# ohsnyt/bzip2-rust

Hardware: AMD Instinct MI355X
Metric: compress MB/s at -9 (900 KB blocks), 1/2/4/8 MI355X; bit-exact vs C bzip2 (higher is better)
Workload: dtype u8; 1 GPU; 1024 MiB per GPU synthetic text at -9 (1194 blocks on this rank), BASELINE configs[2]; raw_bytes_total=1073741824, blocks_rank0=1194, compressed_bytes=323302688

## Files before the change

bzip2-rust_amd/csrc/bzx_api.hip:

```cpp
#include <string.h>
#include <chrono>
#include <new>
#include "bzx_host.h"
#include "bzx_wg.h"

extern "C" const char *bzx_version(void) { return "bzx 0.1 (gfx950)"; }

extern "C" const char *bzx_strerror(int code)
{
    switch (code) {
    case BZX_OK: return "ok";
    case BZX_E_NODEVICE: return "no HIP device";
    case BZX_E_PARAM: return "bad parameter";
    case BZX_E_NOMEM: return "out of memory";
    case BZX_E_OUTBUF: return "output buffer too small";
    case BZX_E_HIP: return "HIP runtime error";
    case BZX_E_STATE: return "bad call sequence";
    case BZX_E_DATA: return "damaged or invalid bzip2 data";
    default: return "unknown error";
    }
}

extern "C" const char *bzx_last_error(const bzx_ctx *ctx) { return ctx ? ctx->err.c_str() : ""; }

// ... 989 lines not shown
}

extern "C" int bzx_split_rle1_chunk(bzx_ctx *ctx, const uint8_t *raw, size_t len, int level, int final, uint8_t *blocks_out,
                                    uint32_t nblk_cap, uint32_t *ns, uint32_t *crcs, uint32_t *nblk_out)
{
    auto api_lock_ = ctx_lock(ctx);
    BZX_REFUSE_WHILE_STREAMING(ctx);
    if (!ctx || !blocks_out || !ns || !crcs || !nblk_out || !level_ok(level) || (len && !raw)) return BZX_E_PARAM;
    HIP_TRY(ctx, hipSetDevice(ctx->device));
    *nblk_out = 0;
    std::vector<uint8_t> &carry = ctx->split_carry;
    const size_t total = carry.size() + len;
    uint32_t use = 0;
    uint64_t last_start = 0;
    int rc = split_to_host(ctx, carry.data(), carry.size(), raw, len, level, final, blocks_out, nblk_cap, ns, crcs, &use,
                           &last_start);
    if (rc) return rc;
    std::vector<uint8_t> next;
    if (!final) {
        const size_t ls = (size_t)last_start, cs = carry.size();
        try {
            next.reserve(total - ls);
            if (ls < cs) next.insert(next.end(), carry.begin() + ls, carry.end());
            const size_t from = ls > cs ? ls - cs : 0;
            if (len > from) next.insert(next.end(), raw + from, raw + len);
        } catch (const std::bad_alloc &) {
            return BZX_E_NOMEM;
        }
    }
    carry.swap(next);
    *nblk_out = use;
    return BZX_OK;
}

extern "C" void *bzx_host_alloc(size_t bytes)
{
    void *p = nullptr;
    return hipHostMalloc(&p, bytes ? bytes : 1, BZX_HOST_PORTABLE) == hipSuccess ? p : nullptr;
}
extern "C" void bzx_host_free(void *p)
{
    if (p) (void)hipHostFree(p);
}


#ifdef BZX_DIAG
extern "C" int bzx_dbg_set_stop(bzx_ctx *ctx, uint32_t k)
{
    if (!ctx) return BZX_E_PARAM;
    ctx->B.dbg_stop = k;
    return BZX_OK;
}

extern "C" int bzx_dbg_phase_timers(bzx_ctx *ctx, int enable, unsigned long long out[128])
{
    if (!ctx) return BZX_E_PARAM;
    if (enable && !ctx->d_dbg) {
        if (hipMalloc((void **)&ctx->d_dbg, 128 * sizeof(unsigned long long)) != hipSuccess) return BZX_E_NOMEM;
    }
    if (out && ctx->d_dbg) {
        HIP_TRY(ctx, hipStreamSynchronize(ctx->stream));
        HIP_TRY(ctx, hipMemcpy(out, ctx->d_dbg, 128 * sizeof(unsigned long long), hipMemcpyDeviceToHost));
    }
    if (ctx->d_dbg) HIP_TRY(ctx, hipMemset(ctx->d_dbg, 0, 128 * sizeof(unsigned long long)));
    ctx->B.dbg = enable ? ctx->d_dbg : nullptr;
    return BZX_OK;
}

extern "C" int bzx_dbg_block_times(bzx_ctx *ctx, uint32_t nblk, uint32_t *us_out, uint32_t *n_out, uint32_t *inuse_out)
{
    if (!ctx || !us_out || nblk > ctx->cap_blocks) return BZX_E_PARAM;
    HIP_TRY(ctx, hipStreamSynchronize(ctx->stream));
    HIP_TRY(ctx, hipMemcpy(ctx->h_blk, ctx->B.blk, nblk * sizeof(BzxBlock), hipMemcpyDeviceToHost));
    for (uint32_t b = 0; b < nblk; b++) {
        us_out[b] = ctx->h_blk[b].pad_[1];
        if (n_out) n_out[b] = ctx->h_blk[b].n;
        if (inuse_out) inuse_out[b] = ctx->h_blk[b].n_in_use;
    }
    return BZX_OK;
}
#endif
```

bzip2-rust_amd/csrc/bzx_bsort.hip:

```cpp
#include <hip/hip_runtime.h>
#include "bzx_host.h"
#include "bzx_wg.h"
#include "bzx_pack.h"

#define BS_NT 1024
#define BS_NW (BS_NT / 64)
#ifndef BS_C
#define BS_C 2048
#endif
#define BS_FW (BS_C / 64)
#define BS_ISO (BS_C / 3)
#ifndef BS_ISO_SHIFT
#define BS_ISO_SHIFT 5
#endif
#ifndef BS_BIN1
#define BS_BIN1 15
#endif
#define BS_BIN2 12
#define BS_NBIN1 (1u << BS_BIN1)
#define BS_TAB_WORDS (BS_NBIN1 + (BS_NBIN1 >> 5))
#define BS_MAX_BK 1024
#ifndef BS_MAX_BIG
#define BS_MAX_BIG 512
#endif
#define SP_U 4
#ifndef BS_MAX_DEPTH
#define BS_MAX_DEPTH 511
#endif
#ifndef BS_MAX_SPLITS
#define BS_MAX_SPLITS 1024
#endif
#ifndef BS_ROUNDS
#define BS_ROUNDS 4
#endif
#ifndef BS_KEYBITS
#define BS_KEYBITS 32
#endif
#define BS_TINY 64
#define BS_MED 512
#define REC_IDX(r) ((uint32_t)((r) >> 12) & 0xFFFFFu)
#define REC_PREV(r) ((uint32_t)((r) >> 4) & 0xFFu)
#define W_POS_MASK 0x3FFFull

static_assert(BS_C <= 16384, "bucket capacity");

#ifdef BZX_DIAG
__shared__ unsigned long long s_diag[128];
#define DIAG_T0()                                                             \
    unsigned long long t_last_ = 0;                                           \
    if (B.dbg && threadIdx.x == 0) {                                          \
        for (int i_ = 0; i_ < 128; i_++) s_diag[i_] = 0;                      \
        t_last_ = wall_clock64();                                             \
    }                                                                         \
    (void)t_last_;
#define DIAG_STAMP(slot)                                                      \
    do {                                                                      \
        if (B.dbg && threadIdx.x == 0) {                                      \
            const unsigned long long now_ = wall_clock64();                   \
            s_diag[slot] += now_ - t_last_;                                   \
            t_last_ = now_;                                                   \
        }                                                                     \
    } while (0)
#define DIAG_COUNT(slot, v)                                                   \
    do {                                                                      \
        if (B.dbg && threadIdx.x == 0) s_diag[slot] += (unsigned long long)(v); \
    } while (0)
#define DIAG_FLUSH()                                                          \
    do {                                                                      \
        if (B.dbg && threadIdx.x == 0)                                        \
            for (int i_ = 0; i_ < 128; i_++)                                  \
                if (s_diag[i_]) atomicAdd(&B.dbg[i_], s_diag[i_]);            \
    } while (0)
#else
#define DIAG_T0() do {} while (0)
#define DIAG_STAMP(slot) do {} while (0)
#define DIAG_COUNT(slot, v) do {} while (0)
#define DIAG_FLUSH() do {} while (0)
#endif

__shared__ uint32_t b_tab[BS_TAB_WORDS + BS_MAX_BK];
__shared__ uint32_t b_start[BS_MAX_BK + 1];
__shared__ uint32_t b_first[BS_MAX_BK + 1];
__shared__ uint32_t b_cur[BS_MAX_BK];
__shared__ uint8_t b_b0[BS_MAX_BK];
__shared__ uint32_t b_inuse[256];
__shared__ uint8_t b_seq[256];
__shared__ uint32_t b_scratch[2 * BS_NW];
__shared__ uint32_t b_lbase[8];
__shared__ uint32_t b_bcast[12];
__shared__ uint32_t b_big[BS_MAX_BIG][3];

#define TAB(b) b_tab[(b) + ((b) >> 5)]

template <int ISO, int PER>
__device__ __forceinline__ void bucket_flags(const uint32_t (&c)[PER], uint32_t bin0, uint32_t excl, uint32_t prevc, uint32_t &fl, uint32_t &nf)
{
    constexpr uint32_t CP = BS_C - ISO;
    uint32_t s = excl, ps = excl - prevc, pc = prevc;
#pragma unroll
    for (int k = 0; k < PER; k++) {
        const bool f = (bin0 + k == 0) || c[k] > (uint32_t)ISO || pc > (uint32_t)ISO || (s / CP != ps / CP);
        fl |= (uint32_t)f << k;
        nf += f;
        ps = s;
        s += c[k];
        pc = c[k];
    }
}

template <int BINS, bool TAB16 = false>
__device__ __forceinline__ uint32_t form_buckets(uint32_t total)
{
    constexpr int PER = BINS / BS_NT;
    const uint32_t tid = threadIdx.x, bin0 = tid * PER;
    uint32_t c[PER], sum = 0, e8 = 0, e6 = 0, e4 = 0;
#pragma unroll
    for (int k = 0; k < PER; k++) {
        c[k] = TAB(bin0 + k);
        sum += c[k];
        const uint32_t m = c[k] <= BS_ISO ? c[k] : 0u;
        e8 += m > BS_C / 8 ? m : 0u;
        e6 += m > BS_C / 6 ? m : 0u;
        e4 += m > BS_C / 4 ? m : 0u;
    }
    const uint32_t prevc = tid ? TAB(bin0 - 1) : 0u;
    if (__any(e8 != 0)) {
// ... 428 lines not shown
{
    const uint32_t tid = threadIdx.x, lvl = B.deep_lvl;
    const uint32_t listed = B.counters[BZX_CTR_DEEP_CNT + lvl];
    const uint32_t n_items = listed < B.deep_cap ? listed : B.deep_cap;
    if (n_items == 0) return;
    DIAG_T0();
    const BzxDeepItem *list = reinterpret_cast<const BzxDeepItem *>(B.deep_list) + (size_t)(lvl & 1u) * B.deep_cap;
    for (;;) {
        if (tid == 0) b_bcast[0] = atomicAdd(&B.counters[BZX_CTR_DEEP_FETCH + lvl], 1u);
        __syncthreads();
        const uint32_t i = b_bcast[0];
        __syncthreads();
        if (i >= n_items) break;
        const BzxDeepItem d = list[i];
        if (d.cnt == 0) continue;
        const uint32_t b = d.blk;
        if (__atomic_load_n(&B.blk[b].status, __ATOMIC_RELAXED) & BZX_ST_REDO) continue;
        const uint32_t n = B.blk[b].n, bits = d.dbits >> 16;
        const size_t sb = BZX_SLAB(B, b);
        const uint8_t *__restrict__ P = B.pk + sb * BZX_PK_STRIDE;
        uint64_t *__restrict__ rec_a = B.rec_a + sb * BZX_MAX_N;
        uint64_t *__restrict__ rec_b = B.rec_b + sb * BZX_MAX_N;
        if (tid == 0) {
            b_bcast[3] = 1;
            b_bcast[4] = 0;
            b_big[0][0] = d.st;
            b_big[0][1] = d.cnt;
            b_big[0][2] = d.dbits & 0xFFFFu;
        }
        __syncthreads();
        const bool ok = deep_process(B, b, (b - B.blk_first) / B.blk_step, n, bits, P, rec_a, rec_b, 0, 1,
                                     lvl + 1 < BZX_DEEP_LEVELS ? (int)lvl + 1 : -1);
        if (!ok && tid == 0) block_redo(B, b);
        __syncthreads();
    }
    DIAG_FLUSH();
}

#ifndef SK_NT
#define SK_NT 256
#endif
#define SK_NW (SK_NT / 64)
#define BS_E (BS_C / SK_NT)
#define SK_DB 8
#define SK_ND (1u << SK_DB)
static_assert(BS_C % SK_NT == 0 && BS_E >= 1 && BS_E <= 8, "bucket capacity");

__shared__ uint64_t s_x[BS_C];
__shared__ __attribute__((aligned(16))) uint64_t s_w[BS_C + 4];
__shared__ __attribute__((aligned(16))) uint32_t s_cnt[SK_NW][SK_ND];
__shared__ uint32_t s_dbase[SK_ND];
__shared__ uint32_t s_part[4];
__shared__ uint64_t s_f[BS_FW + 1];
__shared__ uint32_t s_med[BS_C / BS_TINY + 1];
__shared__ uint32_t s_large[BS_C / BS_MED + 1];
__shared__ uint32_t s_rc[2][4];
__shared__ uint32_t s_bc[8];
__shared__ uint32_t s_m[2];
__shared__ uint32_t s_red[SK_NW][4];

__device__ __forceinline__ uint32_t uni(uint32_t v) { return bzx_uni(v); }
__device__ __forceinline__ uint32_t tid_here() { return bzx_tid_here(); }
__device__ __forceinline__ BzxBucket uni(BzxBucket b)
{
    BzxBucket r;
    r.blk = uni(b.blk);
    r.start = uni(b.start);
    r.cnt = uni(b.cnt);
    if (r.cnt >> 31) r.cnt = 0;
    r.dbits = uni(b.dbits);
    return r;
}

__device__ __forceinline__ void wave_rank(uint32_t *wc, uint32_t d, bool valid, uint32_t lane, uint32_t &old, uint32_t &rank)
{
    uint64_t m = __ballot(valid);
    uint32_t plo = (uint32_t)m, phi = (uint32_t)(m >> 32);
#pragma unroll
    for (int b = 0; b < SK_DB; b++) {
        const uint32_t mask = 0u - ((d >> b) & 1u);
        m = __ballot((d >> b) & 1u);
        plo &= ~((uint32_t)m ^ mask);
        phi &= ~((uint32_t)(m >> 32) ^ mask);
    }
    const uint64_t peers = ((uint64_t)phi << 32) | plo;
    rank = (uint32_t)__popcll(peers & ((1ull << lane) - 1ull));
    old = wc[d];
    lds_order();
    if (valid && rank == 0) atomicAdd(&wc[d], (uint32_t)__popcll(peers));
    lds_order();
}

__device__ __attribute__((noinline)) void wg_radix_sort(uint32_t base, uint32_t cnt, int lo, int hi)
{
    uint64_t *A = s_w + base;
    const uint32_t tid = threadIdx.x, lane = bzx_lane(), wave = bzx_wave();
    const uint32_t rows = (cnt + SK_NT - 1) / SK_NT, chunk = rows * 64;
    if (tid == 0) {
        s_bc[5] = 0;
        s_bc[6] = 0;
    }
    __syncthreads();
    {
        const uint64_t a0 = A[0];
        uint64_t d = 0;
#pragma unroll
// ... 20 lines not shown
        uint32_t old[BS_E], rk[BS_E];
#pragma unroll
        for (uint32_t j = 0; j < BS_E; j++) {
            const uint32_t e = wave * chunk + j * 64 + lane;
            v[j] = j < rows && e < cnt ? A[e] : 0ull;
        }
#pragma unroll
        for (uint32_t j = 0; j < BS_E; j++) {
            const uint32_t e = wave * chunk + j * 64 + lane;
            wave_rank(wc, (uint32_t)(v[j] >> shift) & (SK_ND - 1), j < rows && e < cnt, lane, old[j], rk[j]);
        }
        __syncthreads();
        {
            constexpr uint32_t SK_DK = SK_ND > SK_NT ? SK_ND / SK_NT : 1u;
            if (tid * SK_DK < SK_ND) {
                uint32_t tot[SK_DK], sum = 0;
#pragma unroll
                for (uint32_t i = 0; i < SK_DK; i++) {
                    uint32_t run = 0;
#pragma unroll
                    for (int w = 0; w < SK_NW; w++) {
                        const uint32_t t = s_cnt[w][tid * SK_DK + i];
                        s_cnt[w][tid * SK_DK + i] = run;
                        run += t;
                    }
                    tot[i] = run;
                    sum += run;
                }
                const uint32_t incl = bzx_wave_incl_sum(sum);
                uint32_t run = incl - sum;
#pragma unroll
                for (uint32_t i = 0; i < SK_DK; i++) {
                    s_dbase[tid * SK_DK + i] = run;
                    run += tot[i];
                }
                if (lane == 63) s_part[wave] = incl;
            }
        }
        __syncthreads();
        const uint32_t p1 = s_part[0], p2 = p1 + s_part[1], p3 = p2 + s_part[2];
#pragma unroll
        for (uint32_t j = 0; j < BS_E; j++) {
            const uint32_t e = wave * chunk + j * 64 + lane;
            if (j < rows && e < cnt) {
                const uint32_t d = (uint32_t)(v[j] >> shift) & (SK_ND - 1);
                const uint32_t q = SK_ND > SK_NT ? 0u : d >> 6;
                A[s_dbase[d] + (q == 0 ? 0u : q == 1 ? p1 : q == 2 ? p2 : p3) + wc[d] + old[j] + rk[j]] = v[j];
            }
        }
        __syncthreads();
    }
}

__device__ __attribute__((noinline)) void wg_radix_sort_opt(uint32_t cnt, int lo, int hi)
{
    uint64_t *A = s_x;
    const uint32_t lane = bzx_lane(), wave = bzx_wave();
    const uint32_t rows = (cnt + SK_NT - 1) / SK_NT, chunk = rows * 64;
    __syncthreads();
    uint64_t diff;
    {
        uint32_t o0 = 0, o1 = 0, a0 = ~0u, a1 = ~0u;
#pragma unroll
        for (int w = 0; w < SK_NW; w++) {
            o0 |= s_red[w][0];
            o1 |= s_red[w][1];
            a0 &= s_red[w][2];
            a1 &= s_red[w][3];
        }
        diff = ((uint64_t)(o1 & ~a1) << 32) | (o0 & ~a0);
    }
    uint32_t *wc = s_cnt[wave];
    uint32_t *wb = reinterpret_cast<uint32_t *>(s_w) + wave * SK_ND;
    for (int shift = lo; shift < hi; shift += SK_DB) {
        if (((diff >> shift) & (uint64_t)(SK_ND - 1)) == 0) continue;
#pragma unroll
        for (uint32_t i = 0; i < SK_ND / 64; i++) wc[i * 64 + lane] = 0;
        lds_order();
        uint64_t v[BS_E];
        uint32_t old[BS_E];
#pragma unroll
        for (uint32_t j = 0; j < BS_E; j++) {
            const uint32_t e = wave * chunk + j * 64 + lane;
            v[j] = j < rows && e < cnt ? A[e] : 0ull;
        }
#pragma unroll
        for (uint32_t j = 0; j < BS_E; j++) {
            const uint32_t e = wave * chunk + j * 64 + lane;
            old[j] = bzx_lds_ticket(&wc[(uint32_t)(v[j] >> shift) & (SK_ND - 1)], j < rows && e < cnt);
        }
        __syncthreads();
        {
            static_assert(SK_ND == 4 * 64, "four digits per lane");
            uint32_t mine[4], tot[4], sum = 0;
#pragma unroll
            for (uint32_t i = 0; i < 4; i++) mine[i] = tot[i] = 0;
#pragma unroll
            for (uint32_t w = 0; w < SK_NW; w++) {
                const uint4 c = *reinterpret_cast<const uint4 *>(&s_cnt[w][4 * lane]);
                const uint32_t cc[4] = {c.x, c.y, c.z, c.w};
#pragma unroll
                for (uint32_t i = 0; i < 4; i++) {
                    if (w < wave) mine[i] += cc[i];
                    tot[i] += cc[i];
                }
            }
#pragma unroll
            for (uint32_t i = 0; i < 4; i++) sum += tot[i];
            uint32_t run = bzx_wave_incl_sum(sum) - sum;
            uint4 o;
            o.x = run + mine[0];
            run += tot[0];
            o.y = run + mine[1];
            run += tot[1];
            o.z = run + mine[2];
            run += tot[2];
            o.w = run + mine[3];
            *reinterpret_cast<uint4 *>(&wb[4 * lane]) = o;
        }
        lds_order();
#pragma unroll
        for (uint32_t j = 0; j < BS_E; j++) {
            const uint32_t e = wave * chunk + j * 64 + lane;
            if (j < rows && e < cnt) A[wb[(uint32_t)(v[j] >> shift) & (SK_ND - 1)] + old[j]] = v[j];
        }
        __syncthreads();
    }
}

template <bool TICKETS>
__device__ __attribute__((noinline)) void wave_radix_sort(uint32_t base, uint32_t s, int lo, int hi)
{
    constexpr uint32_t ROWS = BS_MED / 64;
    uint64_t *A = s_w + base;
    uint32_t *wc = s_cnt[bzx_wave()];
    const uint32_t lane = bzx_lane();
    const uint32_t rows = (s + 63u) / 64u;
    uint64_t v[ROWS];
    uint64_t diff = 0;
    {
        const uint64_t a0 = A[0];
#pragma unroll
        for (uint32_t j = 0; j < ROWS; j++) {
            const uint32_t e = j * 64 + lane;
            v[j] = e < s ? A[e] : 0ull;
            if (e < s) diff |= v[j] ^ a0;
        }
#pragma unroll
        for (int sh = 32; sh > 0; sh >>= 1) diff |= __shfl_xor(diff, sh);
    }
    for (int shift = lo; shift < hi; shift += SK_DB) {
        if (((diff >> shift) & (uint64_t)(SK_ND - 1)) == 0) continue;
#pragma unroll
        for (uint32_t i = 0; i < SK_ND / 64; i++) wc[i * 64 + lane] = 0;
        lds_order();
        uint32_t old[ROWS], rk[ROWS];
#pragma unroll
        for (uint32_t j = 0; j < ROWS; j++) {
            old[j] = rk[j] = 0;
            if (j < rows) {
                if (TICKETS) old[j] = bzx_lds_ticket(&wc[(uint32_t)(v[j] >> shift) & (SK_ND - 1)], j * 64 + lane < s);
                else wave_rank(wc, (uint32_t)(v[j] >> shift) & (SK_ND - 1), j * 64 + lane < s, lane, old[j], rk[j]);
            }
        }
        {
            uint32_t c[SK_ND / 64], sum = 0;
#pragma unroll
            for (uint32_t i = 0; i < SK_ND / 64; i++) {
                c[i] = wc[(SK_ND / 64) * lane + i];
                sum += c[i];
            }
            uint32_t run = bzx_wave_incl_sum(sum) - sum;
            lds_order();
#pragma unroll
            for (uint32_t i = 0; i < SK_ND / 64; i++) {
                wc[(SK_ND / 64) * lane + i] = run;
                run += c[i];
            }
        }
        lds_order();
#pragma unroll
        for (uint32_t j = 0; j < ROWS; j++)
            if (j * 64 + lane < s) A[wc[(uint32_t)(v[j] >> shift) & (SK_ND - 1)] + old[j] + rk[j]] = v[j];
        lds_order();
#pragma unroll
        for (uint32_t j = 0; j < ROWS; j++) {
            const uint32_t e = j * 64 + lane;
            v[j] = e < s ? A[e] : 0ull;
        }
        lds_order();
    }
}

__device__ __forceinline__ uint32_t fbit(uint32_t p) { return (uint32_t)(s_f[p >> 6] >> (p & 63u)) & 1u; }
__device__ __forceinline__ void fset(uint32_t p) { atomicOr((unsigned long long *)&s_f[p >> 6], 1ull << (p & 63u)); }

__device__ __forceinline__ bool tiny_bounds(uint32_t p, uint32_t &gs, uint32_t &ge)
{
    const uint32_t wi = p >> 6, bi = p & 63u;
    uint64_t w = s_f[wi] & (~0ull >> (63u - bi));
    if (w) {
        gs = wi * 64 + 63u - (uint32_t)__builtin_clzll(w);
    } else {
        if (wi == 0) return false;
        w = s_f[wi - 1];
        if (!w) return false;
        gs = (wi - 1) * 64 + 63u - (uint32_t)__builtin_clzll(w);
    }
    w = bi == 63u ? 0ull : s_f[wi] & (~0ull << (bi + 1u));
    if (w) {
        ge = wi * 64 + (uint32_t)__builtin_ctzll(w);
    } else {
        w = s_f[wi + 1];
        if (!w) return false;
        ge = (wi + 1) * 64 + (uint32_t)__builtin_ctzll(w);
    }
    return ge - gs <= BS_TINY;
}

__device__ __forceinline__ void mark_changes(uint32_t base, uint32_t s, int lo, uint32_t t, uint32_t step)
{
    for (uint32_t e = 1 + t; e < s; e += step)
        if ((s_w[base + e] >> lo) != (s_w[base + e - 1] >> lo)) fset(base + e);
}

__device__ __forceinline__ bool any_big(uint32_t base, uint32_t s, uint32_t t, uint32_t step)
{
    bool big = false;
    for (uint32_t e = t; e < s; e += step) {
        uint32_t gs, ge;
        big |= !tiny_bounds(base + e, gs, ge);
    }
    return big;
}

__device__ __forceinline__ void wave_sort_mark(uint32_t base, uint32_t s, int lo, uint32_t lane)
{
    wave_radix_sort<true>(base, s, lo, 64);
    lds_order();
    uint32_t diff = 0;
    bool bad = false;
    for (uint32_t e = 1 + lane, k = 0; e < s; e += 64, k++) {
        const uint64_t a = s_w[base + e] >> lo, b = s_w[base + e - 1] >> lo;
        bad |= a < b;
        diff |= (uint32_t)(a != b) << k;
    }
// ... 122 lines not shown
                for (uint32_t k = 0; k < 4; k++) {
                    const bool in = i + k < sz;
                    r += in && wq[k] < my[j];
                    rk += in && wq[k] < myc;
                }
            }
            if (sz) dst_[j] = (a_ + r) | (r != rk ? 0u : 0x80000000u);
        }
    }
    __syncthreads();
}

__device__ __forceinline__ void place_ranked(const uint32_t (&dst_)[BS_E], const uint64_t (&my)[BS_E])
{
#pragma unroll
    for (uint32_t j = 0; j < BS_E; j++) {
        if (dst_[j] != 0xFFFFFFFFu) {
            const uint32_t q = dst_[j] & 0x7FFFFFFFu;
            s_w[q] = my[j];
            if ((dst_[j] >> 31) && !fbit(q)) fset(q);
        }
    }
    __syncthreads();
}

#define LIST(which, i) (reinterpret_cast<uint16_t *>(s_x)[4u * (i) + 2u + (which)])

template <bool ALL>
__device__ __attribute__((noinline)) void list_tied(uint32_t n, uint32_t from, uint32_t to)
{
    const uint32_t tid = tid_here(), lane = tid & 63u;
    const uint32_t nrow = (n + SK_NT - 1) / SK_NT;
#pragma unroll
    for (uint32_t j = 0; j < BS_E; j++) {
        if (j < nrow) {
            const uint32_t i = j * SK_NT + tid;
            uint32_t p = 0;
            bool t = false;
            if (i < n) {
                p = ALL ? i : (uint32_t)LIST(from, i);
                t = !(fbit(p) && fbit(p + 1));
            }
            const uint64_t mk = __ballot(t);
            if (mk) {
                uint32_t base = 0;
                if (lane == 0) base = atomicAdd(&s_m[to], (uint32_t)__popcll(mk));
                base = bzx_bcast0(base);
                if (t) LIST(to, base + (uint32_t)__popcll(mk & ((1ull << lane) - 1ull))) = (uint16_t)p;
            }
        }
    }
}

__device__ __forceinline__ bool initial_sort(uint32_t cnt)
{
    const uint32_t tid = tid_here(), lane = tid & 63u, wave = tid >> 6;
    uint64_t fm[BS_E];
    wg_radix_sort_opt(cnt, 64 - BS_KEYBITS, 64);
    int bad = 0;
#pragma unroll
    for (uint32_t j = 0; j < BS_E; j++) {
        const uint32_t p = j * SK_NT + tid;
        s_w[p] = p;
        const uint64_t kp = s_x[p] >> (64 - BS_KEYBITS), kq = p ? s_x[p - 1] >> (64 - BS_KEYBITS) : 0ull;
        const bool f = p >= cnt || p == 0 || kp != kq;
        bad |= p < cnt && p > 0 && kp < kq;
        fm[j] = __ballot(f);
        if (lane == 0) s_f[j * SK_NW + wave] = fm[j];
    }
    if (tid == 0) s_f[BS_FW] = ~0ull;
    if (__syncthreads_or(bad)) return false;
#pragma unroll
    for (uint32_t j = 0; j < BS_E; j++) {
        const uint64_t mk = tied_mask(fm[j], s_f[j * SK_NW + wave + 1]);
        if (mk) {
            uint32_t base = 0;
            if (lane == 0) base = atomicAdd(&s_m[0], (uint32_t)__popcll(mk));
            base = bzx_bcast0(base);
            if ((mk >> lane) & 1ull) LIST(0, base + (uint32_t)__popcll(mk & ((1ull << lane) - 1ull))) = (uint16_t)(j * SK_NT + tid);
        }
    }
    return true;
}

__device__ __attribute__((noinline)) uint32_t wave_rounds(const uint8_t *__restrict__ P, uint32_t bits, uint32_t nbits, uint32_t m,
                                                          uint32_t lpar, uint32_t round, uint32_t dcur)
{
    const uint32_t lane = bzx_lane();
    for (;; round++) {
        if (m == 0) return dcur;
        if (!(round < BS_ROUNDS && dcur < nbits)) return dcur | 0x80000000u;
        const bool has = lane < m;
        uint32_t p = 0, gs = 0, ge = 0;
        uint64_t my = 0;
        if (has) {
            p = LIST(lpar, lane);
            const uint32_t pos = (uint32_t)(s_w[p] & W_POS_MASK);
            uint32_t x = REC_IDX(s_x[pos]) * bits + dcur;
            if (x >= nbits) x -= nbits;
            my = (pk_window_bit(P, x) & ~W_POS_MASK) | pos;
            tiny_bounds(p, gs, ge);
        }
        lds_order();
        if (has) s_w[p] = my;
        lds_order();
        uint32_t r = 0, rk = 0;
        const uint64_t myc = my & ~W_POS_MASK;
        const uint32_t sz = ge - gs;
        for (uint32_t i = 0; __ballot(i < sz); i++) {
            if (i < sz) {
                const uint64_t o = s_w[gs + i];
                r += o < my;
                rk += o < myc;
            }
        }
        lds_order();
        if (has) {
            const uint32_t q = gs + r;
            s_w[q] = my;
            if (r == rk && !fbit(q)) fset(q);
        }
        lds_order();
        const bool t = has && !(fbit(p) && fbit(p + 1));
        const uint64_t mk = __ballot(t);
        if (t) LIST(lpar ^ 1u, (uint32_t)__popcll(mk & ((1ull << lane) - 1ull))) = (uint16_t)p;
        lds_order();
        m = (uint32_t)__popcll(mk);
        lpar ^= 1u;
        dcur += 50;
    }
}

#ifndef SK_WAVES_PER_SIMD
#define SK_WAVES_PER_SIMD 4
#endif
#ifdef BZX_HIP_EMU
#define BS_LOAD_REC(p) (*(p))
#else
#define BS_LOAD_REC(p) __builtin_nontemporal_load(p)
#endif
__device__ __forceinline__ void bsort_body(const BzxBatch &B)
{
    const uint32_t tid0 = threadIdx.x;
    if (B.bsort_mode == 1 && B.counters[BZX_CTR_RESUME] == 0) return;
    DIAG_T0();
    const uint32_t G = gridDim.x >> 3;
    const uint32_t cap8 = B.bk_cap >> 3, lx = blockIdx.x & 7u;
    const uint32_t n_lx = B.counters[BZX_CTR_BK_LIST0 + lx] < cap8 ? B.counters[BZX_CTR_BK_LIST0 + lx] : cap8;
    const uint32_t n_items = lx * cap8 + n_lx;
    uint32_t idx = lx * cap8 + (blockIdx.x >> 3);
    BzxBucket it = {0, 0, 0, 0}, nit = {0, 0, 0, 0};
    if (idx < n_items) it = uni(B.bk_list[idx]);
    if (idx + G < n_items) nit = uni(B.bk_list[idx + G]);
    uint64_t nxt[BS_E];
    uint32_t n_cur = 0, st_cur = 0;
    if (it.cnt) {
        const uint64_t *__restrict__ src = ((it.start >> 31) ? B.rec_b : B.rec_a) + BZX_SLAB(B, it.blk) * BZX_MAX_N +
                                           (it.start & 0x7fffffffu);
#pragma unroll
        for (uint32_t j = 0; j < BS_E; j++) nxt[j] = j * SK_NT + tid0 < it.cnt ? BS_LOAD_REC(src + j * SK_NT + tid0) : ~0ull;
        n_cur = uni(B.blk[it.blk].n);
        st_cur = uni(__atomic_load_n(&B.blk[it.blk].status, __ATOMIC_RELAXED));
    }
    for (; idx < n_items; idx += G) {
        BzxBucket nit2 = {0, 0, 0, 0};
        if (idx + 2 * G < n_items) nit2 = B.bk_list[idx + 2 * G];
        uint32_t tid = tid_here(), lane = tid & 63u, wave = tid >> 6;
        const uint32_t b = it.blk, cnt = it.cnt;
        const uint32_t start = it.start & 0x7fffffffu, bits = it.dbits >> 16, depth0 = it.dbits & 0xFFFFu;
        const uint8_t *__restrict__ P = B.pk + BZX_SLAB(B, b) * BZX_PK_STRIDE;
        const uint32_t nbits = n_cur * bits;
        const bool skip = cnt == 0 || (cnt >> 31) || (st_cur & BZX_ST_REDO) || (B.bsort_mode == 1 && !(st_cur & BZX_ST_RESUME));
        DIAG_STAMP(64);
        if (!skip) {
            uint32_t o0 = 0, o1 = 0, a0 = ~0u, a1 = ~0u;
#pragma unroll
            for (uint32_t j = 0; j < BS_E; j++) {
                s_x[j * SK_NT + tid] = nxt[j];
                if (j * SK_NT + tid < cnt) {
                    o0 |= (uint32_t)nxt[j];
                    o1 |= (uint32_t)(nxt[j] >> 32);
                    a0 &= (uint32_t)nxt[j];
                    a1 &= (uint32_t)(nxt[j] >> 32);
                }
            }
            o0 = bzx_wave_incl_or(o0);
            o1 = bzx_wave_incl_or(o1);
            a0 = bzx_wave_incl_and(a0);
            a1 = bzx_wave_incl_and(a1);
            if (lane == 63) {
                s_red[wave][0] = o0;
                s_red[wave][1] = o1;
                s_red[wave][2] = a0;
                s_red[wave][3] = a1;
            }
        }
        uint32_t n_nx = 0, st_nx = 0;
#define PREFETCH_NEXT()                                                                                                   \
        if (nit.cnt) {                                                                                                    \
            const uint64_t *__restrict__ src = ((nit.start >> 31) ? B.rec_b : B.rec_a) + BZX_SLAB(B, nit.blk) * BZX_MAX_N + \
                                               (nit.start & 0x7fffffffu);                                                 \
            const uint32_t tp_ = tid_here();                                                                              \
            _Pragma("unroll") for (uint32_t j = 0; j < BS_E; j++) nxt[j] = j * SK_NT + tp_ < nit.cnt ? BS_LOAD_REC(src + j * SK_NT + tp_) : ~0ull; \
            n_nx = B.blk[nit.blk].n;                                             \
            st_nx = __atomic_load_n(&B.blk[nit.blk].status, __ATOMIC_RELAXED);                                            \
        }
        if (skip) {
            PREFETCH_NEXT();
            it = nit;
            nit = uni(nit2);
            n_cur = uni(n_nx);
            st_cur = uni(st_nx);
            continue;
        }
        if (tid < 4) s_rc[0][tid] = 0;
        if (tid < 2) s_m[tid] = 0;
        DIAG_STAMP(65);
        if (!initial_sort(cnt)) {
            if (tid == 0) {
                atomicAdd(&B.counters[BZX_CTR_STAT0 + 15], 1u);
                block_redo(B, b);
            }
            PREFETCH_NEXT();
            __syncthreads();
            it = nit;
            nit = uni(nit2);
            n_cur = uni(n_nx);
            st_cur = uni(st_nx);
            continue;
        }
        DIAG_STAMP(67);

        uint32_t dcur = depth0 + BS_KEYBITS;
        bool fail = false;
        uint32_t lpar = 0;
        __syncthreads();
        DIAG_STAMP(73);
        for (uint32_t round = 0;; round++) {
            tid = tid_here();
            lane = tid & 63u;
            wave = tid >> 6;
            const uint32_t par = round & 1u;
            const uint32_t m = uni(s_m[lpar]);
            if (m == 0) break;
            if (m <= 64) {
                DIAG_COUNT(89, 1);
                if (wave == 0) {
                    dcur = wave_rounds(P, bits, nbits, m, lpar, round, dcur);
                    if (lane == 0) s_bc[3] = dcur;
                }
                __syncthreads();
                dcur = uni(s_bc[3]);
                fail = dcur >> 31;
                dcur &= 0x7FFFFFFFu;
                DIAG_STAMP(70);
                break;
            }
            if (!(round < BS_ROUNDS && dcur < nbits)) {
                DIAG_COUNT(round >= BS_ROUNDS ? 84 : 85, 1);
                fail = true;
                break;
            }
            DIAG_COUNT(80, 1);
            DIAG_COUNT(88, m);
            const uint32_t nrow = (m + SK_NT - 1) / SK_NT;
            uint32_t amask = 0, hmask = 0;
            uint32_t pq[BS_E], xa[BS_E];
#pragma unroll
            for (uint32_t j = 0; j < BS_E; j++) {
                pq[j] = 0;
                xa[j] = 0;
// ... 11 lines not shown
            for (uint32_t j = 0; j < BS_E; j++) {
                if ((amask >> j) & 1u) {
                    uint32_t x = REC_IDX(s_x[pq[j] >> 16]) * bits + dcur;
                    if (x >= nbits) x -= nbits;
                    xa[j] = x;
                }
            }
            uint64_t g[BS_E];
#pragma unroll
            for (uint32_t j = 0; j < BS_E; j++) g[j] = ((amask >> j) & 1u) ? pk_window_bit(P, xa[j]) : 0ull;
            const auto rank_of = [&](uint32_t j) { return pq[j] & 0xFFFFu; };
            list_big_groups(hmask, par, rank_of);
#pragma unroll
            for (uint32_t j = 0; j < BS_E; j++)
                if ((amask >> j) & 1u) s_w[pq[j] & 0xFFFFu] = (g[j] & ~W_POS_MASK) | (uint64_t)(pq[j] >> 16);
            if (tid == 0) {
                s_rc[par ^ 1u][0] = s_rc[par ^ 1u][1] = s_rc[par ^ 1u][2] = s_rc[par ^ 1u][3] = 0;
                s_m[lpar ^ 1u] = 0;
            }
            __syncthreads();
            DIAG_STAMP(68);
            const uint32_t nmed = s_rc[par][1], nlarge = s_rc[par][2];
            if (nmed | nlarge) {
                DIAG_COUNT(86, nmed);
                DIAG_COUNT(87, nlarge);
                sort_listed_groups(par, nmed, nlarge, tid, lane);
                DIAG_STAMP(69);
            }
            tid = tid_here();
            lane = tid & 63u;
            wave = tid >> 6;
            uint32_t dst_[BS_E];
            uint64_t my[BS_E];
            rank_tiny_groups(amask, nrow, rank_of, dst_, my);
            DIAG_STAMP(70);
            place_ranked(dst_, my);
            DIAG_STAMP(71);
            list_tied<false>(m, lpar, lpar ^ 1u);
            __syncthreads();
            DIAG_STAMP(73);
            lpar ^= 1u;
            dcur += 50;
        }
        PREFETCH_NEXT();
        tid = tid_here();
        if (fail || B.bsort_mode == 1) {
            uint64_t *__restrict__ sax = B.rec_a + BZX_SLAB(B, b) * BZX_MAX_N + start;
            const uint32_t rk = uni(B.blk[b].n_selectors);
            uint32_t *__restrict__ isa0 = rank_array(B, rk, 0), *__restrict__ isa1 = rank_array(B, rk, 1);
#pragma unroll
            for (uint32_t j = 0; j < BS_E; j++) {
                const uint32_t p = j * SK_NT + tid;
                if (p < cnt) {
                    const uint32_t rot = REC_IDX(s_x[(uint32_t)(s_w[p] & W_POS_MASK)]);
                    const uint32_t f0 = fbit(p);
                    sax[p] = (uint64_t)rot | ((uint64_t)f0 << 32);
                    if (isa0) {
                        const uint32_t head = f0 ? p : group_start(p);
                        isa0[rot] = start + head;
                        if (f0 && fbit(p + 1)) isa1[rot] = start + head;
                    }
                }
            }
            if (fail) {
                uint32_t *__restrict__ cl = reinterpret_cast<uint32_t *>(B.rec_b + BZX_SLAB(B, b) * BZX_MAX_N + start);
                uint64_t mk[BS_E];
                lane = tid & 63u;
                wave = tid >> 6;
#pragma unroll
                for (uint32_t j = 0; j < BS_E; j++) mk[j] = tied_mask(s_f[j * SK_NW + wave], s_f[j * SK_NW + wave + 1]);
                slot_counts_publish(mk, BS_E);
                __syncthreads();
                uint32_t before[BS_E];
                const uint32_t total = slot_counts_sum(BS_E, before);
#pragma unroll
                for (uint32_t j = 0; j < BS_E; j++) {
                    if ((mk[j] >> lane) & 1ull) {
                        const uint32_t p = j * SK_NT + tid;
                        const uint32_t rot = REC_IDX(s_x[(uint32_t)(s_w[p] & W_POS_MASK)]);
                        cl[before[j] + (uint32_t)__popcll(mk[j] & ((1ull << lane) - 1ull))] = p | (fbit(p) << 11) | (rot << 12);
                    }
                }
                if (tid == 0) {
                    atomicMin(&B.blk[b].n_mtf, dcur / bits);
                    B.bk_list[idx].cnt = cnt | 0x80000000u;
                    const uint32_t ri = atomicAdd(&B.counters[BZX_CTR_RK_ITEMS], 1u);
                    B.rk_list[ri] = idx;
                    B.rk_list[B.bk_cap + ri] = total;
                    atomicAdd(&B.counters[BZX_CTR_RK_OPEN], 1u);
                    atomicAdd(&B.blk[b].n_groups, 1u);
                    if ((atomicOr(&B.blk[b].status, BZX_ST_RESUME) & BZX_ST_RESUME) == 0)
                        B.resume_list[atomicAdd(&B.counters[BZX_CTR_RESUME], 1u)] = b;
                }
            }
        }
        {
            constexpr uint32_t OUT_E = 8;
            uint8_t *__restrict__ L = B.bwt + BZX_SLAB(B, b) * BZX_BLK_STRIDE + start;
            const uint32_t p0 = tid * OUT_E;
            if (p0 < cnt) {
                const uint32_t rot = tid >> 2;
                uint32_t pos[OUT_E];
#pragma unroll
                for (uint32_t k = 0; k < OUT_E; k++) pos[k] = (uint32_t)(s_w[p0 + ((k + rot) & (OUT_E - 1))] & W_POS_MASK);
                uint64_t bytes = 0;
#pragma unroll
                for (uint32_t k = 0; k < OUT_E; k++) {
                    const uint32_t kk = (k + rot) & (OUT_E - 1);
                    const uint32_t r = reinterpret_cast<const uint32_t *>(s_x)[2u * pos[k]];
                    bytes |= (uint64_t)REC_PREV(r) << (8 * kk);
                    if (p0 + kk < cnt && REC_IDX(r) == 0) B.blk[b].orig_ptr = start + p0 + kk;
                }
                if (p0 + OUT_E <= cnt) {
                    __builtin_memcpy(L + p0, &bytes, 8);
                } else {
                    for (uint32_t k = 0; p0 + k < cnt; k++) L[p0 + k] = (uint8_t)(bytes >> (8 * k));
                }
            }
            DIAG_COUNT(83, 1);
        }
        __syncthreads();
        DIAG_STAMP(72);
        it = nit;
        nit = uni(nit2);
        n_cur = uni(n_nx);
        st_cur = uni(st_nx);
    }
    DIAG_FLUSH();
}

__global__ __launch_bounds__(SK_NT, SK_WAVES_PER_SIMD) void bzx_bsort_kernel(BzxBatch B) { bsort_body(B); }
__global__ __launch_bounds__(SK_NT, SK_WAVES_PER_SIMD) void bzx_bfill_kernel(BzxBatch B) { bsort_body(B); }

#define RK_CHUNK 16
struct RkMeta {
    uint32_t bi, T, blk, start, cnt, n, rk, h0;
};
__shared__ RkMeta s_meta[RK_CHUNK];

__device__ __forceinline__ uint32_t rk_fetch_chunk(const BzxBatch &B, uint32_t n_items, uint32_t &open)
{
    __shared__ uint32_t s_fetch[2];
    __syncthreads();
    if (threadIdx.x < 64) {
        uint32_t base = 0;
        if (threadIdx.x == 0) base = atomicAdd(&B.counters[B.rk_fetch], (uint32_t)RK_CHUNK);
        base = __shfl(base, 0);
        const uint32_t i = base + threadIdx.x;
        bool op = false;
        if (threadIdx.x < RK_CHUNK && i < n_items) {
            RkMeta m;
            m.bi = B.rk_list[i];
            m.T = B.rk_list[B.bk_cap + i];
            const BzxBucket it = B.bk_list[m.bi];
            op = !(it.dbits >> 31);
            m.blk = it.blk;
            m.start = it.start & 0x7fffffffu;
            m.cnt = it.cnt & 0x7fffffffu;
            m.n = B.blk[it.blk].n;
            m.rk = B.blk[it.blk].n_selectors;
            m.h0 = B.blk[it.blk].n_mtf;
            s_meta[threadIdx.x] = m;
        }
        const uint64_t m = __ballot(op);
        if (threadIdx.x == 0) {
            s_fetch[0] = base;
            s_fetch[1] = (uint32_t)m;
        }
    }
    __syncthreads();
    open = s_fetch[1];
    return s_fetch[0];
}

__shared__ uint32_t s_stall[2 * BS_FW];

__device__ __forceinline__ void rank_round_wave(const BzxBatch &B, uint32_t i)
{
    const uint32_t lane = bzx_lane(), wave = bzx_wave();
    const RkMeta &mt = s_meta[i & (RK_CHUNK - 1)];
// ... 543 lines not shown
```

bzip2-rust_amd/csrc/bzx_device.h:

```cpp
#pragma once
#include <stdint.h>
#include <stddef.h>

#define BZX_MAX_N 900000u
#define BZX_BLK_STRIDE 900096u
#define BZX_MAX_ALPHA 258
#define BZX_G_SIZE 50
#define BZX_N_ITERS 4
#define BZX_MAX_SEL 18002
#define BZX_SEL_STRIDE 18048

#define BZX_IN_RAW (1ull << 63)
#define BZX_ST_PERIODIC 1u
#define BZX_ST_REDO 2u
#define BZX_ST_RESUME 4u
#define BZX_ST_DC_RANDOMISED 0x400u
#define DC_ERR_HEADER 0x100u
#define DC_ERR_DATA 0x200u
#define DC_SKIP 0x800u
#define DC_MAGIC_BLOCK 0x314159265359ull
#define DC_MAGIC_EOS 0x177245385090ull
#ifndef RK_ROUNDS
#define RK_ROUNDS 11
#endif
#define RK_COARSE 0x80000000u
#define BZX_PK_STRIDE 900352u
#ifndef BZX_BK_PER_BLOCK
#define BZX_BK_PER_BLOCK 2048u
#endif

#define BZX_CTR_PERIODIC 5
#define BZX_CTR_BK_LIST0 40
#ifndef BZX_DEEP_LEVELS
#define BZX_DEEP_LEVELS 2
#endif
#define BZX_DEEP_PER_BLOCK 128u
#define BZX_CTR_DEEP_CNT 48
#define BZX_CTR_DEEP_FETCH 56
#define BZX_CTR_GIANT_CNT (BZX_CTR_DEEP_CNT + BZX_DEEP_LEVELS)
#define BZX_CTR_GIANT_FETCH (BZX_CTR_DEEP_FETCH + BZX_DEEP_LEVELS)
#define BZX_CTR_BK_FETCH 9
#define BZX_CTR_REDO 10
#define BZX_CTR_SPLIT_FETCH 11
#define BZX_CTR_REDO_FETCH 12
#define BZX_CTR_RESUME 13
#define BZX_CTR_RESUME_FETCH 14
#define BZX_CTR_RK_ITEMS 32
#define BZX_CTR_RK_OPEN 33
#define BZX_CTR_RK_FETCH 64
#define BZX_N_COUNTERS 192
#define BZX_CTR_RESUME_LEFT 34
#define BZX_CTR_STAT0 16

struct BzxBucket {
    uint32_t blk;
    uint32_t start;
    uint32_t cnt;
    uint32_t dbits;
};

struct BzxBlock {
    uint64_t in_off;
    uint32_t n;
    uint32_t crc;
    uint32_t orig_ptr;
    uint32_t status;
    uint32_t n_mtf;
    uint32_t n_in_use;
    uint32_t n_groups;
    uint32_t n_selectors;
    uint64_t bits;
    uint64_t out_bit;
    uint32_t sec_bits[4];
    uint32_t pad_[2];
    uint64_t pack_word;
};

struct BzxSortWs {
    uint64_t *u0;
    uint64_t *u1;
    uint32_t *s0;
    uint32_t *s1;
    uint32_t *isa;
    uint32_t *sa;
};

struct BzxBatch {
    BzxBlock *blk;
    uint32_t nblk;
    uint32_t blk_first;
    uint32_t blk_step;
    uint32_t ctr_bwt;
    uint32_t packed;
    uint32_t *counters;
    uint32_t *plist;
    const uint8_t *in;
    const uint8_t *raw;
    uint8_t *bwt;
    uint8_t *rank;
    uint32_t *hpos;
    uint32_t hpos_stride;
    uint16_t *mtfv;
    uint32_t *freq;
// ... 93 lines not shown
```

Baseline: 29770 MB/s.

## Feed bucket-sort records from registers and skip identity position writes

The radix sort now takes the prefetched records as register arguments, so the initial store of all records to shared memory and the reload in the first pass go away. The global prefetch layout changes to wave-chunked rows so each thread already holds the elements the sort expects. A per-word 'tied' bitmap (s_t) is added so s_w position entries are written only for tied positions, and readers fall back to the identity index otherwise, which cuts LDS writes. A debug per-workgroup timer export is also added. The cost is more shared memory and a branch on every position lookup.

```diff
diff --git a/bzip2-rust_amd/csrc/bzx_api.hip b/bzip2-rust_amd/csrc/bzx_api.hip
--- a/bzip2-rust_amd/csrc/bzx_api.hip
+++ b/bzip2-rust_amd/csrc/bzx_api.hip
@@ -1065,11 +1065,20 @@
     return BZX_OK;
 }
 
+extern "C" int bzx_dbg_wg_times(bzx_ctx *ctx, unsigned long long out[BZX_DBG_WG])
+{
+    if (!ctx || !out || !ctx->d_dbg) return BZX_E_PARAM;
+    HIP_TRY(ctx, hipStreamSynchronize(ctx->stream));
+    HIP_TRY(ctx, hipMemcpy(out, ctx->d_dbg + 128, BZX_DBG_WG * sizeof(unsigned long long), hipMemcpyDeviceToHost));
+    return BZX_OK;
+}
+
 extern "C" int bzx_dbg_phase_timers(bzx_ctx *ctx, int enable, unsigned long long out[128])
 {
     if (!ctx) return BZX_E_PARAM;
     if (enable && !ctx->d_dbg) {
-        if (hipMalloc((void **)&ctx->d_dbg, 128 * sizeof(unsigned long long)) != hipSuccess) return BZX_E_NOMEM;
+        if (hipMalloc((void **)&ctx->d_dbg, (128 + BZX_DBG_WG) * sizeof(unsigned long long)) != hipSuccess) return BZX_E_NOMEM;
+        if (hipMemset(ctx->d_dbg, 0, (128 + BZX_DBG_WG) * sizeof(unsigned long long)) != hipSuccess) return BZX_E_NOMEM;
     }
     if (out && ctx->d_dbg) {
         HIP_TRY(ctx, hipStreamSynchronize(ctx->stream));
diff --git a/bzip2-rust_amd/csrc/bzx_bsort.hip b/bzip2-rust_amd/csrc/bzx_bsort.hip
--- a/bzip2-rust_amd/csrc/bzx_bsort.hip
+++ b/bzip2-rust_amd/csrc/bzx_bsort.hip
@@ -71,7 +71,16 @@
             for (int i_ = 0; i_ < 128; i_++)                                  \
                 if (s_diag[i_]) atomicAdd(&B.dbg[i_], s_diag[i_]);            \
     } while (0)
+#define DIAG_WG_TIME()                                                        \
+    do {                                                                      \
+        if (B.dbg && threadIdx.x == 0 && B.bsort_mode == 0 && blockIdx.x < BZX_DBG_WG) { \
+            unsigned long long sum_ = 0;                                      \
+            for (int i_ = 64; i_ < 74; i_++) sum_ += s_diag[i_];              \
+            B.dbg[128 + blockIdx.x] = sum_;                                   \
+        }                                                                     \
+    } while (0)
 #else
+#define DIAG_WG_TIME() do {} while (0)
 #define DIAG_T0() do {} while (0)
 #define DIAG_STAMP(slot) do {} while (0)
 #define DIAG_COUNT(slot, v) do {} while (0)
@@ -606,6 +615,7 @@
 __shared__ uint32_t s_dbase[SK_ND];
 __shared__ uint32_t s_part[4];
 __shared__ uint64_t s_f[BS_FW + 1];
+__shared__ uint64_t s_t[BS_FW];
 __shared__ uint32_t s_med[BS_C / BS_TINY + 1];
 __shared__ uint32_t s_large[BS_C / BS_MED + 1];
 __shared__ uint32_t s_rc[2][4];
@@ -732,11 +742,24 @@
     }
 }
 
-__device__ __attribute__((noinline)) void wg_radix_sort_opt(uint32_t cnt, int lo, int hi)
-{
+#ifdef BZX_HIP_EMU
+extern "C" {
+unsigned bzx_emu_bsort_nopass = 0;
+}
+#define BS_NOPASS_HOOK() do { if (threadIdx.x == 0) bzx_emu_bsort_nopass++; } while (0)
+#else
+#define BS_NOPASS_HOOK() do {} while (0)
+#endif
+
+__device__ __attribute__((noinline)) void wg_radix_sort_opt(uint32_t cnt, int lo, int hi, uint64_t x0, uint64_t x1, uint64_t x2, uint64_t x3,
+                                                            uint64_t x4, uint64_t x5, uint64_t x6, uint64_t x7)
+{
+    static_assert(BS_E == 8, "one parameter per row");
     uint64_t *A = s_x;
     const uint32_t lane = bzx_lane(), wave = bzx_wave();
     const uint32_t rows = (cnt + SK_NT - 1) / SK_NT, chunk = rows * 64;
+    uint64_t v[BS_E] = {x0, x1, x2, x3, x4, x5, x6, x7};
+    bool first = true;
     __syncthreads();
     uint64_t diff;
     {
@@ -757,13 +780,15 @@
 #pragma unroll
         for (uint32_t i = 0; i < SK_ND / 64; i++) wc[i * 64 + lane] = 0;
         lds_order();
-        uint64_t v[BS_E];
         uint32_t old[BS_E];
-#pragma unroll
-        for (uint32_t j = 0; j < BS_E; j++) {
-            const uint32_t e = wave * chunk + j * 64 + lane;
-            v[j] = j < rows && e < cnt ? A[e] : 0ull;
-        }
+        if (!first) {
+#pragma unroll
+            for (uint32_t j = 0; j < BS_E; j++) {
+                const uint32_t e = wave * chunk + j * 64 + lane;
+                v[j] = j < rows && e < cnt ? A[e] : 0ull;
+            }
+        }
+        first = false;
 #pragma unroll
         for (uint32_t j = 0; j < BS_E; j++) {
             const uint32_t e = wave * chunk + j * 64 + lane;
@@ -806,6 +831,15 @@
         }
         __syncthreads();
     }
+    if (first) {
+        BS_NOPASS_HOOK();
+#pragma unroll
+        for (uint32_t j = 0; j < BS_E; j++) {
+            const uint32_t e = wave * chunk + j * 64 + lane;
+            if (j < rows && e < cnt) A[e] = v[j];
+        }
+        __syncthreads();
+    }
 }
 
 template <bool TICKETS>
@@ -872,6 +906,10 @@
     }
 }
 
+__device__ __forceinline__ uint32_t pos_of(uint32_t p)
+{
+    return ((s_t[p >> 6] >> (p & 63u)) & 1ull) ? (uint32_t)(s_w[p] & W_POS_MASK) : p;
+}
 __device__ __forceinline__ uint32_t fbit(uint32_t p) { return (uint32_t)(s_f[p >> 6] >> (p & 63u)) & 1u; }
 __device__ __forceinline__ void fset(uint32_t p) { atomicOr((unsigned long long *)&s_f[p >> 6], 1ull << (p & 63u)); }
 
@@ -1100,16 +1138,15 @@
     }
 }
 
-__device__ __forceinline__ bool initial_sort(uint32_t cnt)
+__device__ __forceinline__ bool initial_sort(uint32_t cnt, const uint64_t (&rec)[BS_E])
 {
     const uint32_t tid = tid_here(), lane = tid & 63u, wave = tid >> 6;
     uint64_t fm[BS_E];
-    wg_radix_sort_opt(cnt, 64 - BS_KEYBITS, 64);
+    wg_radix_sort_opt(cnt, 64 - BS_KEYBITS, 64, rec[0], rec[1], rec[2], rec[3], rec[4], rec[5], rec[6], rec[7]);
     int bad = 0;
 #pragma unroll
     for (uint32_t j = 0; j < BS_E; j++) {
         const uint32_t p = j * SK_NT + tid;
-        s_w[p] = p;
         const uint64_t kp = s_x[p] >> (64 - BS_KEYBITS), kq = p ? s_x[p - 1] >> (64 - BS_KEYBITS) : 0ull;
         const bool f = p >= cnt || p == 0 || kp != kq;
         bad |= p < cnt && p > 0 && kp < kq;
@@ -1121,11 +1158,15 @@
 #pragma unroll
     for (uint32_t j = 0; j < BS_E; j++) {
         const uint64_t mk = tied_mask(fm[j], s_f[j * SK_NW + wave + 1]);
+        if (lane == 0) s_t[j * SK_NW + wave] = mk;
         if (mk) {
             uint32_t base = 0;
             if (lane == 0) base = atomicAdd(&s_m[0], (uint32_t)__popcll(mk));
             base = bzx_bcast0(base);
-            if ((mk >> lane) & 1ull) LIST(0, base + (uint32_t)__popcll(mk & ((1ull << lane) - 1ull))) = (uint16_t)(j * SK_NT + tid);
+            if ((mk >> lane) & 1ull) {
+                LIST(0, base + (uint32_t)__popcll(mk & ((1ull << lane) - 1ull))) = (uint16_t)(j * SK_NT + tid);
+                s_w[j * SK_NT + tid] = j * SK_NT + tid;
+            }
         }
     }
     return true;
@@ -1187,6 +1228,8 @@
 #else
 #define BS_LOAD_REC(p) __builtin_nontemporal_load(p)
 #endif
+#define BS_CHUNK_OF(cnt) ((((cnt) + SK_NT - 1) / SK_NT) * 64u)
+#define BS_ROW_OF(j, chunk, e0, cnt) ((j) * 64u < (chunk) && (e0) + (j) * 64u < (cnt))
 __device__ __forceinline__ void bsort_body(const BzxBatch &B)
 {
     const uint32_t tid0 = threadIdx.x;
@@ -1205,8 +1248,9 @@
     if (it.cnt) {
         const uint64_t *__restrict__ src = ((it.start >> 31) ? B.rec_b : B.rec_a) + BZX_SLAB(B, it.blk) * BZX_MAX_N +
                                            (it.start & 0x7fffffffu);
-#pragma unroll
-        for (uint32_t j = 0; j < BS_E; j++) nxt[j] = j * SK_NT + tid0 < it.cnt ? BS_LOAD_REC(src + j * SK_NT + tid0) : ~0ull;
+        const uint32_t chunk = BS_CHUNK_OF(it.cnt), e0 = (tid0 >> 6) * chunk + (tid0 & 63u);
+#pragma unroll
+        for (uint32_t j = 0; j < BS_E; j++) nxt[j] = BS_ROW_OF(j, chunk, e0, it.cnt) ? BS_LOAD_REC(src + e0 + j * 64) : ~0ull;
         n_cur = uni(B.blk[it.blk].n);
         st_cur = uni(__atomic_load_n(&B.blk[it.blk].status, __ATOMIC_RELAXED));
     }
@@ -1222,10 +1266,10 @@
         DIAG_STAMP(64);
         if (!skip) {
             uint32_t o0 = 0, o1 = 0, a0 = ~0u, a1 = ~0u;
+            const uint32_t chunk = BS_CHUNK_OF(cnt), e0 = wave * chunk + lane;
 #pragma unroll
             for (uint32_t j = 0; j < BS_E; j++) {
-                s_x[j * SK_NT + tid] = nxt[j];
-                if (j * SK_NT + tid < cnt) {
+                if (BS_ROW_OF(j, chunk, e0, cnt)) {
                     o0 |= (uint32_t)nxt[j];
                     o1 |= (uint32_t)(nxt[j] >> 32);
                     a0 &= (uint32_t)nxt[j];
@@ -1249,7 +1293,8 @@
             const uint64_t *__restrict__ src = ((nit.start >> 31) ? B.rec_b : B.rec_a) + BZX_SLAB(B, nit.blk) * BZX_MAX_N + \
                                                (nit.start & 0x7fffffffu);                                                 \
             const uint32_t tp_ = tid_here();                                                                              \
-            _Pragma("unroll") for (uint32_t j = 0; j < BS_E; j++) nxt[j] = j * SK_NT + tp_ < nit.cnt ? BS_LOAD_REC(src + j * SK_NT + tp_) : ~0ull; \
+            const uint32_t ch_ = BS_CHUNK_OF(nit.cnt), e0_ = (tp_ >> 6) * ch_ + (tp_ & 63u);                              \
+            _Pragma("unroll") for (uint32_t j = 0; j < BS_E; j++) nxt[j] = BS_ROW_OF(j, ch_, e0_, nit.cnt) ? BS_LOAD_REC(src + e0_ + j * 64) : ~0ull; \
             n_nx = B.blk[nit.blk].n;                                             \
             st_nx = __atomic_load_n(&B.blk[nit.blk].status, __ATOMIC_RELAXED);                                            \
         }
@@ -1264,7 +1309,7 @@
         if (tid < 4) s_rc[0][tid] = 0;
         if (tid < 2) s_m[tid] = 0;
         DIAG_STAMP(65);
-        if (!initial_sort(cnt)) {
+        if (!initial_sort(cnt, nxt)) {
             if (tid == 0) {
                 atomicAdd(&B.counters[BZX_CTR_STAT0 + 15], 1u);
                 block_redo(B, b);
@@ -1382,7 +1427,7 @@
             for (uint32_t j = 0; j < BS_E; j++) {
                 const uint32_t p = j * SK_NT + tid;
                 if (p < cnt) {
-                    const uint32_t rot = REC_IDX(s_x[(uint32_t)(s_w[p] & W_POS_MASK)]);
+                    const uint32_t rot = REC_IDX(s_x[pos_of(p)]);
                     const uint32_t f0 = fbit(p);
                     sax[p] = (uint64_t)rot | ((uint64_t)f0 << 32);
                     if (isa0) {
@@ -1407,7 +1452,7 @@
                 for (uint32_t j = 0; j < BS_E; j++) {
                     if ((mk[j] >> lane) & 1ull) {
                         const uint32_t p = j * SK_NT + tid;
-                        const uint32_t rot = REC_IDX(s_x[(uint32_t)(s_w[p] & W_POS_MASK)]);
+                        const uint32_t rot = REC_IDX(s_x[pos_of(p)]);
                         cl[before[j] + (uint32_t)__popcll(mk[j] & ((1ull << lane) - 1ull))] = p | (fbit(p) << 11) | (rot << 12);
                     }
                 }
@@ -1430,9 +1475,14 @@
             const uint32_t p0 = tid * OUT_E;
             if (p0 < cnt) {
                 const uint32_t rot = tid >> 2;
+                const uint32_t tb = reinterpret_cast<const uint8_t *>(s_t)[tid];
                 uint32_t pos[OUT_E];
 #pragma unroll
-                for (uint32_t k = 0; k < OUT_E; k++) pos[k] = (uint32_t)(s_w[p0 + ((k + rot) & (OUT_E - 1))] & W_POS_MASK);
+                for (uint32_t k = 0; k < OUT_E; k++) {
+                    const uint32_t kk = (k + rot) & (OUT_E - 1);
+                    pos[k] = p0 + kk;
+                    if ((tb >> kk) & 1u) pos[k] = (uint32_t)(s_w[p0 + kk] & W_POS_MASK);
+                }
                 uint64_t bytes = 0;
 #pragma unroll
                 for (uint32_t k = 0; k < OUT_E; k++) {
@@ -1456,6 +1506,7 @@
         n_cur = uni(n_nx);
         st_cur = uni(st_nx);
     }
+    DIAG_WG_TIME();
     DIAG_FLUSH();
 }
 
diff --git a/bzip2-rust_amd/csrc/bzx_device.h b/bzip2-rust_amd/csrc/bzx_device.h
--- a/bzip2-rust_amd/csrc/bzx_device.h
+++ b/bzip2-rust_amd/csrc/bzx_device.h
@@ -49,6 +49,7 @@
 #define BZX_CTR_RK_OPEN 33
 #define BZX_CTR_RK_FETCH 64
 #define BZX_N_COUNTERS 192
+#define BZX_DBG_WG 2048
 #define BZX_CTR_RESUME_LEFT 34
 #define BZX_CTR_STAT0 16
 
```

Result: slower. 29470 MB/s (-1.0%).
